# segasai/rvspecfit

Hardware: AMD Instinct MI355X
Metric: spectra/sec (CCF+chi2 grid) DESI 3-arm (higher is better)
Workload: dtype f64

## Files before the change

### include/rvsgpu.h

```cpp
#ifndef RVSGPU_H
#define RVSGPU_H
#include <stdint.h>

#ifdef __cplusplus
extern "C" {
#endif

#define RVS_E_ARG (-1)
#define RVS_E_LAUNCH (-2)

#define RVS_ST_SPLINE_RANGE 0x1
#define RVS_ST_SPLINE_GRID 0x2
#define RVS_ST_NONFINITE 0x4
#define RVS_ST_CHOL_FALLBACK 0x8
#define RVS_ST_OUTSIDE_NAN 0x10
#define RVS_ST_CCF_FAILED 0x20
#define RVS_ST_ALLMASKED 0x40
#define RVS_ST_QUAD_ASSERT 0x80
#define RVS_ST_ILLCOND 0x100
#define RVS_ST_NONPOS_MEDIAN 0x200
#define RVS_ST_RBF_NOTPD 0x400

#define RVS_ABI_VERSION 18
int rvs_abi_version(void);
// ... 80 lines not shown
int rvs_chisq_grid(const double *lam, const double *polysT, const double *work,
                   int npix, int npoly, int S, const double *knots,
                   const double *coef, int ntp, int Tn, int log_step,
                   const int32_t *job_spec, const int32_t *job_templ, int J,
                   const double *vels, int64_t vel_stride, int Nv,
                   const double *penalty, double badchi, double beta,
                   int pack_min_jobs, double *out, int32_t *status,
                   void *stream);

int64_t rvs_chisq_work_size_g(int npix, int S, int G);
int rvs_chisq_prepare_g(const double *lam, const double *spec,
                        const double *espec, int npix, int S, int G,
                        const double *knots_host3, int log_step, double espec_sys,
                        double *work, void *stream);
int rvs_chisq_grid_g(const double *lam, const double *polysT, const double *work,
                     int npix, int npoly, int S, const int32_t *grid_id, int G,
                     int64_t polys_stride, const double *knots,
                     const double *coef, int ntp, int Tn, int log_step,
                     const int32_t *job_spec, const int32_t *job_templ, int J,
                     const double *vels, int64_t vel_stride, int Nv,
                     const double *penalty, double badchi, double beta,
                     int pack_min_jobs, const double *pen_scale, double *out,
                     int32_t *status, void *stream);

int rvs_chisq_grid_resol(const double *lam, const double *polysT,
                         const double *work, int npix, int npoly, int S,
                         const double *knots, const double *coef, int ntp,
                         int Tn, int log_step, const double *taps, int nd,
                         int64_t taps_stride, const int32_t *job_spec,
                         const int32_t *job_templ, int J, const double *vels,
                         int64_t vel_stride, int Nv, const double *penalty,
                         double badchi, double beta, double *out,
                         int32_t *status, void *stream);
int rvs_chisq_grid_resol_g(const double *lam, const double *polysT,
                           const double *work, int npix, int npoly, int S,
                           const int32_t *grid_id, int G, int64_t polys_stride,
                           const double *knots, const double *coef, int ntp,
                           int Tn, int log_step, const double *taps, int nd,
                           int64_t taps_stride, const int32_t *job_spec,
                           const int32_t *job_templ, int J, const double *vels,
                           int64_t vel_stride, int Nv, const double *penalty,
                           double badchi, double beta, const double *pen_scale,
                           double *out, int32_t *status, void *stream);

int rvs_chisq_full(const double *lam, const double *polysT, const double *spec,
                   const double *espec, const uint8_t *badmask, int npix,
// ... 521 lines not shown
```

### rvspecfit_amd/_lib.py

```python
import ctypes
import os

import torch

_HERE = os.path.dirname(os.path.abspath(__file__))
LIB_PATH = os.path.join(_HERE, 'librvsgpu.so')

P = ctypes.c_void_p
I = ctypes.c_int
L = ctypes.c_int64
D = ctypes.c_double
U = ctypes.c_uint32

SIGNATURES = {
    'rvs_abi_version': (I, []),
    'rvs_option_set': (I, [ctypes.c_char_p, I]),
    'rvs_option_get': (I, [ctypes.c_char_p, P]),
    'rvs_template_polylinear': (I, [P, L, I, P, P, P, I, P, P, U, I, P, I, P, P,
                                    P, P, P]),
    'rvs_template_polylinear_grad': (I, [P, L, I, P, P, P, I, P, P, U, I, P, I, P,
                                         P, P, P, P]),
    'rvs_template_tri': (I, [P, I, P, P, P, I, I, U, I, P, I, P, P, P, P, P]),
    'rvs_template_tri_buckets': (I, [P, I, P, P, P, I, I, U, I, P, P, I, P, P, P,
                                     P, P]),
    'rvs_template_tri_grad': (I, [P, I, P, P, P, I, I, U, I, P, I, P, P, P, P, P]),
    'rvs_template_tri_buckets_grad': (I, [P, I, P, P, P, I, I, U, I, P, P, I, P, P,
                                          P, P, P]),
    'rvs_vsini_convolve': (I, [P, P, P, D, D, I, I, P, P]),
    'rvs_vsini_convolve_grad': (I, [P, P, P, D, D, I, I, I, P, P]),
    'rvs_spline_factors': (I, [P, I, P, P]),
    'rvs_spline_factors_len': (ctypes.c_int64, [I]),
    'rvs_spline_construct': (I, [P, P, I, I, I, P, P, P]),
    'rvs_spline_eval': (I, [P, P, I, I, P, I, I, P, P, P, P]),
    'rvs_chisq_work_size': (L, [I, I]),
    'rvs_chisq_work_size_g': (L, [I, I, I]),
    'rvs_chisq_prepare_g': (I, [P, P, P, I, I, I, P, I, D, P, P]),
    'rvs_chisq_grid_g': (I, [P, P, P, I, I, I, P, I, L, P, P, I, I, I, P, P, I, P, L,
                             I, P, D, D, I, P, P, P, P]),
    'rvs_chisq_prepare': (I, [P, P, P, I, I, P, I, D, P, P]),
    'rvs_chisq_grid': (I, [P, P, P, I, I, I, P, P, I, I, I, P, P, I, P, L, I, P,
                           D, D, I, P, P, P]),
    'rvs_chisq_grid_resol': (I, [P, P, P, I, I, I, P, P, I, I, I, P, I, L, P, P,
                                 I, P, L, I, P, D, D, P, P, P]),
    'rvs_chisq_grid_resol_g': (I, [P, P, P, I, I, I, P, I, L, P, P, I, I, I, P, I, L,
                                   P, P, I, P, L, I, P, D, D, P, P, P, P]),
    'rvs_chisq_full': (I, [P, P, P, P, P, I, I, I, P, P, I, I, I, I, I, P, P, I,
                           P, D, I, P, I, L, P, P, P, P, P, P, P, P]),
    'rvs_chisq_full_g': (I, [P, P, P, P, P, I, I, I, P, P, I, I, I, I, I, P, P, I,
                             P, D, I, P, I, L, P, P, P, P, P, P, P, P, I, L, P]),
    'rvs_chisq_continuum_work_size': (L, [I, I]),
    'rvs_chisq_continuum_g': (I, [P, P, P, P, P, I, I, I, P, P, P, P, P, P, I, L,
                                  P]),
    'rvs_chisq_continuum': (I, [P, P, P, P, P, I, I, I, P, P, P, P, P, P]),
    'rvs_chisq_point_work_size': (L, [I, I]),
    'rvs_chisq_point': (I, [P, I, I, P, P, I, P, D, P, P, P, P]),
    'rvs_chisq_point_grad_work_size': (L, [I, I, I]),
    'rvs_chisq_point_grad': (I, [P, I, I, I, P, P, I, P, D, P, P, P, P, P, P]),
    'rvs_chisq_point_fisher_work_size': (L, [I, I, I]),
    'rvs_chisq_point_fisher': (I, [P, I, I, I, P, P, I, P, D, P, P, P, P, P, P, P]),
    'rvs_chisq_point_grad_resol_work_size': (L, [I, I, I]),
    'rvs_chisq_point_grad_resol': (I, [P, I, I, I, P, P, I, P, D, P, P, P, P, P, P]),
# ... 309 lines not shown
```

### rvspecfit_amd/csrc/chisq.hip

```cpp
#include "common.h"
#include <type_traits>

extern "C" int64_t rvs_chisq_work_size_g(int npix, int S, int G) {
  return (int64_t)G * npix + 4ll * S * npix + 2ll * S + 2ll * G * npix;
}
extern "C" int64_t rvs_chisq_work_size(int npix, int S) {
  return rvs_chisq_work_size_g(npix, S, 1);
}

__global__ void __launch_bounds__(256)
    chisq_prepare_kernel(const double *__restrict__ lam,
                         const double *__restrict__ spec,
                         const double *__restrict__ espec, int npix, int S, int G,
                         double x0, double inv_step, int log_step,
                         double espec_sys, double *__restrict__ work) {
  __shared__ double red[8];
  const int s = blockIdx.x;
  double2 *W = reinterpret_cast<double2 *>(work + (int64_t)G * npix);
  double *scal = work + (int64_t)G * npix + 2ll * S * npix;
  double2 *X = reinterpret_cast<double2 *>(scal + 2ll * S);
  if (s >= S) {
    const double lx0 = log(x0);
    const double *lg = lam + (int64_t)(s - S) * npix;
    double *pixa = work + (int64_t)(s - S) * npix;
// ... 71 lines not shown
    if constexpr ((R & 1) != 0) asm volatile("" : "+s"(d));
  }
  __device__ __forceinline__ double get(int i) const {
    if (N8 >= 1 && i < 8) return a0[i];
    if (N8 >= 2 && i < 16) return a1[i - 8];
    int j = i - 8 * N8;
    if ((R & 4) != 0) {
      if (j < 4) return b[j];
      j -= 4;
    }
    if ((R & 2) != 0) {
      if (j < 2) return c[j];
      j -= 2;
    }
    return d;
  }
};
typedef int cg_v4i __attribute__((ext_vector_type(4)));
typedef int cg_v2i __attribute__((ext_vector_type(2)));
__device__ cg_v4i cg_sbl128(cg_v4i rsrc, int vindex, int voffset, int soffset,
                            int aux) __asm("llvm.amdgcn.struct.buffer.load.v4i32");
__device__ cg_v2i cg_sbl64(cg_v4i rsrc, int vindex, int voffset, int soffset,
                           int aux) __asm("llvm.amdgcn.struct.buffer.load.v2i32");
__device__ __forceinline__ cg_v4i cg_rsrc(const void *p, unsigned stride,
                                          unsigned nrec) {
  const unsigned long long a = (unsigned long long)p;
  cg_v4i r;
  r.x = (int)(unsigned)a;
  r.y = (int)(((unsigned)(a >> 32) & 0xffffu) | (stride << 16));
  r.z = (int)nrec;
  r.w = 0x00020000;
  return r;
}
template <int I, int N, class F>
__device__ __forceinline__ void cg_static_for(F &&f) {
  if constexpr (I < N) {
    f(std::integral_constant<int, I>{});
    cg_static_for<I + 1, N>(f);
  }
}
__device__ __forceinline__ void cg_sload2(double &d, const double *p) { d = *p; }
__device__ __forceinline__ void cg_sload4(cg_d2 &d, const double2 *p) {
  typedef double d2u __attribute__((ext_vector_type(2), aligned(8)));
  d = *reinterpret_cast<const d2u *>(p);
}

#define CG_WAVES(P) ((P) <= 10 ? 3 : 2)
__host__ __device__ constexpr int cg_split(int P) {
  if (P <= 13) return P;
  int pa = 1;
  while (pa < P && pa * (pa + 3) < P * (P + 3) / 2) pa++;
  return pa;
}

template <int P, bool TAIL>
__device__ __forceinline__ void
    chisq_grid_body(const int bx, const int by, const double *__restrict__ lam,
                      const double *__restrict__ polysT,
                      const double *__restrict__ work, int npix, int S,
                      const double *__restrict__ knots,
                      const double4 *__restrict__ coef, int ntp, int log_step,
                      const int32_t *__restrict__ job_spec,
                      const int32_t *__restrict__ job_templ, int J,
                      const double *__restrict__ vels, int64_t vel_stride,
                      int Nv, int iv0, int lpj,
                      const double *__restrict__ penalty, double badchi,
                      double beta_out, double *__restrict__ out,
                      int32_t *__restrict__ status, const GridSet GS) {
  int j, iv;
  bool active;
  if (TAIL) {
    const int64_t g = (int64_t)bx * 64 + threadIdx.x;
    j = (int)(g / lpj);
    iv = iv0 + (int)(g - (int64_t)j * lpj);
    active = j < J;
    if (!active) {
      j = 0;
      iv = iv0;
    }
  } else {
    j = by;
    iv = bx * 64 + threadIdx.x;
    active = iv < iv0;
    if (!active) iv = bx * 64;
  }
  const int s = job_spec ? job_spec[j] : j;
  const int t = job_templ ? job_templ[j] : j;
  double *outp = out + (int64_t)j * Nv;

  const double pen = penalty ? penalty[j] : 0.0;
  const bool unusable = !(pen == pen) || isinf(pen);
  if (GS.pen_scale) badchi *= GS.pen_scale[s];
  if (!TAIL && unusable) {
    if (active) {
      const double base = (beta_out != 0.0) ? beta_out * outp[iv] : 0.0;
      outp[iv] = base + 1000.0 * badchi;
    }
    return;
  }

  int gsel = 0;
  if (!TAIL && GS.gid) gsel = GS.gid[__builtin_amdgcn_readfirstlane(s)];
  gsel = __builtin_amdgcn_readfirstlane(gsel);
  lam += (int64_t)gsel * npix;
  polysT += (int64_t)gsel * GS.polys_stride;
  const double *pixa = work + (int64_t)gsel * npix;
  const double2 *W0 =
      reinterpret_cast<const double2 *>(work + (int64_t)GS.G * npix);
  const uint32_t woff = TAIL ? (uint32_t)s * (uint32_t)npix * 16u : 0u;
  const double2 *W = W0 + (TAIL ? 0 : (int64_t)s * npix);
  const double *scal = work + (int64_t)GS.G * npix + 2ll * S * npix + 2 * s;
  const double4 *cf = coef + (int64_t)t * ntp;

  const double vel = vels[(int64_t)j * vel_stride + iv];
  const double bb = vel / RVS_C_KMS;
  const double f = sqrt((1.0 - bb) / (1.0 + bb));
  const double x0 = knots[0], xlast = knots[ntp - 1];
  double shift;
  if (log_step) {
    const double inv_step = 1.0 / log(knots[1] / x0);
    shift = log(f) * inv_step;
  } else {
    shift = 0;
  }
  const double lin_inv_step = log_step ? 0.0 : 1.0 / (knots[1] - x0);

  int32_t st = 0;
  {
    const double xa = lam[0] * f, xb = lam[npix - 1] * f;
    if (xa < x0 || xb < x0 || xa >= xlast || xb >= xlast)
      st |= RVS_ST_SPLINE_RANGE;
  }
  int npx = npix;
  if (!TAIL && GS.gid) {
    const double last = lam[npix - 1];
    int lo = 0, hi = npix - 1;
    while (lo < hi) {
      const int mid = (lo + hi) >> 1;
      if (lam[mid] < last)
        lo = mid + 1;
      else
        hi = mid;
    }
    npx = __builtin_amdgcn_readfirstlane(lo + 1);
  }

  double acc[P * (P + 1) / 2];
  double av[P];
#pragma unroll
  for (int i = 0; i < P * (P + 1) / 2; i++) acc[i] = 0;
#pragma unroll
  for (int i = 0; i < P; i++) av[i] = 0;

  auto weights = [&](int k) -> double2 {
    if (TAIL)
      return *reinterpret_cast<const double2 *>(
          reinterpret_cast<const char *>(W0 + k) + woff);
    return W[k];
  };
  auto trips = [&](auto log_c, auto i0_c, auto i1_c) {
    constexpr bool LOG = decltype(log_c)::value;
    constexpr int I0 = decltype(i0_c)::value, I1 = decltype(i1_c)::value;
    auto pos_of = [&](double lamk, double pixk, double &x) {
      {
#pragma clang fp contract(off)
        x = lamk * f;
      }
      int pos;
      if (LOG)
        pos = (int)(pixk + shift);
      else
        pos = (int)((x - x0) * lin_inv_step);
      int r;
      asm("v_med3_i32 %0, %1, 0, %2" : "=v"(r) : "v"(pos), "s"(ntp - 2));
      return r;
    };
    const cg_v4i rk = cg_rsrc(knots, 8, (unsigned)ntp);
    const cg_v4i rc = cg_rsrc(cf, 32, (unsigned)ntp);
    auto knot_at = [&](int p) -> double {
      if (!TAIL) {
        const cg_v2i v = cg_sbl64(rk, p, 0, 0, 0);
        return __hiloint2double(v.y, v.x);
      }
      return *reinterpret_cast<const double *>(
          reinterpret_cast<const char *>(knots) + ((uint32_t)p << 3));
    };
    auto rec_at = [&](int p) -> double4 {
      if (!TAIL) {
        const cg_v4i lo = cg_sbl128(rc, p, 0, 0, 0);
        const cg_v4i hi = cg_sbl128(rc, p, 16, 0, 0);
        return make_double4(__hiloint2double(lo.y, lo.x),
                            __hiloint2double(lo.w, lo.z),
                            __hiloint2double(hi.y, hi.x),
                            __hiloint2double(hi.w, hi.z));
      }
      return *reinterpret_cast<const double4 *>(
          reinterpret_cast<const char *>(cf) + ((uint32_t)p << 5));
    };
    double w, u;
    {
      double x;
      const int p0 = pos_of(lam[0], pixa[0], x);
      const double d0 = x - knot_at(p0);
      const double4 c0 = rec_at(p0);
      const double2 w0 = weights(0);
      const double t0 = fma(fma(fma(c0.w, d0, c0.z), d0, c0.y), d0, c0.x);
      w = t0 * t0 * w0.x;
      u = t0 * w0.y;
    }
    const int klast = npx - 1;
    CgRow<P> R0, R1;
    double la0, pa0, la1, pa1;
    R0.load(polysT);
    cg_sload2(la0, lam + min(1, klast));
    cg_sload2(pa0, pixa + min(1, klast));
    asm volatile("" : "+s"(la0), "+s"(pa0));
    R0.pin();
    auto trip = [&](int k, CgRow<P> &Rc, CgRow<P> &Rn, double lac, double pac,
                    double &lan, double &pan) {
      const int k1 = min(k + 1, klast), k2 = min(k + 2, klast);
      Rn.load(polysT + (int64_t)k1 * P);
      cg_d2 wn_s;
      if (!TAIL) cg_sload4(wn_s, W + k1);
      cg_sload2(lan, lam + k2);
      cg_sload2(pan, pixa + k2);
      double xn;
      const int pn = pos_of(lac, pac, xn);
      double kn = knot_at(pn);
      double4 cn = rec_at(pn);
      double2 wn_v;
      if (TAIL) wn_v = weights(k1);
      CG_FENCE();
#pragma unroll
      for (int jj = 0; jj < I1; jj++) {
        const double pj = Rc.get(jj);
        const double pwj = pj * w;
        if (jj >= I0) av[jj] = fma(pj, u, av[jj]);
#pragma unroll
        for (int i = (jj > I0 ? jj : I0); i < I1; i++)
          acc[TRI(i, jj)] = fma(Rc.get(i), pwj, acc[TRI(i, jj)]);
      }
      CG_FENCE();
      asm volatile(""
                   : "+v"(kn), "+v"(cn.x), "+v"(cn.y), "+v"(cn.z), "+v"(cn.w));
      const double dn = xn - kn;
      const double tn = fma(fma(fma(cn.w, dn, cn.z), dn, cn.y), dn, cn.x);
      if (TAIL) {
        asm volatile("" : "+s"(lan), "+s"(pan));
        w = tn * tn * wn_v.x;
        u = tn * wn_v.y;
      } else {
        asm volatile("" : "+s"(lan), "+s"(pan), "+s"(wn_s));
        w = tn * tn * wn_s[0];
        u = tn * wn_s[1];
      }
      Rn.pin();
    };
    int k = 0;
#pragma unroll 1
    for (; k + 1 < npx; k += 2) {
      trip(k, R0, R1, la0, pa0, la1, pa1);
      trip(k + 1, R1, R0, la1, pa1, la0, pa0);
    }
    if (k < npx) trip(k, R0, R1, la0, pa0, la1, pa1);
  };
  constexpr int PS = cg_split(P);
  using c0_t = std::integral_constant<int, 0>;
  using cs_t = std::integral_constant<int, PS>;
  using cp_t = std::integral_constant<int, P>;
  if (log_step) {
    trips(std::true_type{}, c0_t{}, cs_t{});
    if constexpr (PS < P) trips(std::true_type{}, cs_t{}, cp_t{});
  } else {
    trips(std::false_type{}, c0_t{}, cs_t{});
    if constexpr (PS < P) trips(std::false_type{}, cs_t{}, cp_t{});
  }

  bool ok = true;
  double ldet = 0;
  double pmin = 1.79e308, pmax = 0;
#pragma unroll
  for (int i = 0; i < P; i++) {
#pragma unroll
    for (int jj = 0; jj <= i; jj++) {
      double sum = acc[TRI(i, jj)];
#pragma unroll
      for (int k = 0; k < jj; k++) sum -= acc[TRI(i, k)] * acc[TRI(jj, k)];
      if (jj == i) {
        if (!(sum > 0)) ok = false;
        pmin = fmin(pmin, sum);
        pmax = fmax(pmax, sum);
        const double d = sqrt(sum);
        acc[TRI(i, i)] = d;
// ... 54 lines not shown
  unsigned long long c0 = 0, r0 = 0;
  if (blockIdx.x == 4096) {
    c0 = __builtin_readcyclecounter();
    r0 = wall_clock64();
  }
#endif
  if (!TAIL) {
    const int per = 8 * nfull;
    const int g = bx / per, r = bx - g * per;
    by = g * 8 + (r & 7);
    bx = r >> 3;
    if (by >= J) return;
  }
  chisq_grid_body<P, TAIL>(bx, by, lam, polysT, work, npix, S,
                           knots, coef, ntp, log_step, job_spec, job_templ, J,
                           vels, vel_stride, Nv, iv0, lpj, penalty, badchi,
                           beta_out, out, status, GS);
#ifdef CG_CLOCK
  if (blockIdx.x == 4096 && threadIdx.x == 0) {
    cg_clock_dbg[0] = __builtin_readcyclecounter() - c0;
    cg_clock_dbg[1] = wall_clock64() - r0;
  }
#endif
}

#define RES_MAXND 33

template <int P>
__global__ void __launch_bounds__(256, (P <= 10 ? 2 : 1))
    chisq_grid_resol_kernel(const double *__restrict__ lam,
                            const double *__restrict__ polysT,
                            const double *__restrict__ work, int npix, int S,
                            const double *__restrict__ knots,
                            const double4 *__restrict__ coef, int ntp,
                            int log_step, const double *__restrict__ taps,
                            int nd, int64_t taps_stride,
                            const int32_t *__restrict__ job_spec,
                            const int32_t *__restrict__ job_templ,
                            const double *__restrict__ vels, int64_t vel_stride,
                            int Nv, const double *__restrict__ penalty,
                            double badchi, double beta_out,
                            double *__restrict__ out,
                            int32_t *__restrict__ status, GridSet GS) {
  extern __shared__ double ring[];
  const int j = blockIdx.y;
  const int wave_v0 = blockIdx.x * 256 + (threadIdx.x & ~63);
// ... 407 lines not shown
    }
    hipLaunchKernelGGL((chisq_grid_kernel<P, true>),
                       dim3((unsigned)(((int64_t)J * r + 63) / 64)),
                       dim3(64), 0, ts, lam, polysT, work, npix, S, knots, cf,
                       ntp, log_step, job_spec, job_templ, J, vels, vel_stride,
                       Nv, iv0, r, 0, penalty, badchi, beta, out, status, GS);
    RVS_LAUNCH_CHECK();
    if (fk && hipEventRecord(fk->join, fk->side) != hipSuccess)
      return RVS_E_LAUNCH;
  }
  if (nfull > 0) {
    const int64_t nb = (int64_t)((J + 7) / 8) * 8 * nfull;
    if (nb > 0x7fffffffll) return RVS_E_ARG;
    hipLaunchKernelGGL((chisq_grid_kernel<P, false>), dim3((unsigned)nb),
                       dim3(64), 0, st, lam, polysT, work, npix, S, knots, cf,
                       ntp, log_step, job_spec, job_templ, J, vels, vel_stride,
                       Nv, iv0, 64, nfull, penalty, badchi, beta, out, status,
                       GS);
    RVS_LAUNCH_CHECK();
  }
  if (fk && hipStreamWaitEvent(st, fk->join, 0) != hipSuccess)
    return RVS_E_LAUNCH;
  return 0;
}

extern "C" int rvs_chisq_prepare_g(const double *lam, const double *spec,
                                   const double *espec, int npix, int S, int G,
                                   const double *knots_host3, int log_step,
                                   double espec_sys, double *work, void *stream) {
  if (npix < 1 || S < 1 || G < 1 || !work) return RVS_E_ARG;
  const double x0 = knots_host3[0], x1 = knots_host3[1], x2 = knots_host3[2];
  double step, step2;
  if (log_step) {
    step = log(x1 / x0);
    step2 = log(x2 / x1);
  } else {
    step = x1 - x0;
    step2 = x2 - x1;
  }
  if (fabs(step - step2) > 1e-10) return -3;
  hipLaunchKernelGGL(chisq_prepare_kernel, dim3(S + G), dim3(256), 0,
                     rvs_stream(stream), lam, spec, espec, npix, S, G, x0,
                     1.0 / step, log_step, espec_sys, work);
  RVS_LAUNCH_CHECK();
  return 0;
}
// ... 1969 lines not shown
```

### rvspecfit_amd/csrc/options.cpp

```cpp
#include <atomic>
#include <cstdlib>
#include <cstring>
#include <mutex>

#include "options.h"

namespace {
struct OptDef {
  const char *name;
  const char *env;
  int dflt;
};
const OptDef kDefs[RVS_OPT_COUNT] = {
    {"xc_ws", "RVS_XC_WS", 1},
    {"obj_inblk_max", "RVS_OBJ_INBLK_MAX", 768},
    {"obj_sort", "RVS_OBJ_SORT", 1},
    {"nn_pipe", "RVS_NN_PIPE", 1},
    {"nm_split_min", "RVS_NM_SPLIT_MIN", 1024},
    {"nm_spec_max", "RVS_NM_SPEC_MAX", 21},
    {"nm_tail_window", "RVS_NM_TAIL_WINDOW", 16},
};
std::atomic<int> g_val[RVS_OPT_COUNT];
std::once_flag g_once;

void init_table() {
  for (int i = 0; i < RVS_OPT_COUNT; i++) {
    int v = kDefs[i].dflt;
    if (const char *ev = std::getenv(kDefs[i].env))
      v = std::atoi(ev);
    g_val[i].store(v, std::memory_order_relaxed);
  }
}
int find(const char *name) {
  if (!name) return -1;
  for (int i = 0; i < RVS_OPT_COUNT; i++)
    if (!std::strcmp(name, kDefs[i].name)) return i;
  return -1;
}
}

int rvs_opt(int id) {
  std::call_once(g_once, init_table);
  return g_val[id].load(std::memory_order_relaxed);
// ... 17 lines not shown
```

### rvspecfit_amd/csrc/options.h

```cpp
#pragma once
#include "../../include/rvsgpu.h"

enum {
  RVS_OPT_XC_WS,
  RVS_OPT_OBJ_INBLK_MAX,
  RVS_OPT_OBJ_SORT,
  RVS_OPT_NN_PIPE,
  RVS_OPT_NM_SPLIT_MIN,
  RVS_OPT_NM_SPEC_MAX,
  RVS_OPT_NM_TAIL_WINDOW,
  RVS_OPT_COUNT
};
int rvs_opt(int id);
```

### rvspecfit_amd/engine.py

```python
import numpy as np
import torch

from . import _lib
from . import ccf_tables

SPEED_OF_LIGHT = 299792.458

KTIMERS = None


class _ktime:

    def __init__(self, name, units=1):
        self.name, self.units = name, units

    def __enter__(self):
        if KTIMERS is not None:
            self.e0 = torch.cuda.Event(enable_timing=True)
            self.e0.record()

    def __exit__(self, *a):
        if KTIMERS is not None:
            e1 = torch.cuda.Event(enable_timing=True)
            e1.record()
# ... 535 lines not shown
    _lib.check(rc, 'rvs_spline_construct')
    if return_templ:
        return coef, outside, templ
    return coef, outside


def convolve_vsini(lib_or_lam, templ, vsini, eps=0.6):
    L = _lib.lib()
    lam = lib_or_lam.lam if hasattr(lib_or_lam, 'lam') else lib_or_lam
    ratios = lam[1:] / lam[:-1]
    assert np.allclose(ratios, ratios[0]), "Wavelength grid must be logarithmic."
    lnstep = float(np.log(ratios[0]))
    out = torch.empty_like(templ)
    rc = L.rvs_vsini_convolve(_lib.ptr(templ.contiguous()), _lib.ptr(vsini),
                              None, lnstep, float(eps), templ.shape[1],
                              templ.shape[0], _lib.ptr(out), _lib.stream())
    _lib.check(rc, 'rvs_vsini_convolve')
    return out


XCORR_PRUNE = True
import os as _os
CG_PACK_MIN_JOBS = 0


def _arm_resol(arm, ia, resols):
    if resols is not None and resols[ia] is not None:
        if arm.resol is not None:
            raise ValueError('You are not allowed to set resol_param together '
                             'with the resolution of each SpecData')
        return resols[ia]
    return arm.resol


def chisq_grid(batch, libs, coefs, outsides, vels, npoly=5, rbf=True,
               job_spec=None, job_templ=None, espec_sys=0.0,
               outside_penalty=True, out=None, vel_bounds=None, resols=None,
               defer_redo=False):
    L = _lib.lib()
    dev = batch.device
    if job_spec is not None:
        J = job_spec.shape[0]
    elif job_templ is not None:
        J = job_templ.shape[0]
    else:
        J = batch.S
    vels = vels.to(device=dev, dtype=torch.float64).contiguous()
    shared = vels.dim() == 1
    Nv = vels.shape[-1]
    vstride = 0 if shared else Nv
    def by_point_kernel(rows):
        js = job_spec if job_spec is not None else _arange32(0, J, dev)
        jt = job_templ if job_templ is not None else _arange32(0, J, dev)
        vv = vels[None, :].expand(J, Nv) if shared else vels
        if rows is not None:
            js, jt, vv = js[rows], jt[rows], vv[rows]
        n = js.shape[0]
        vv = vv.reshape(-1)
        res = torch.empty(n * Nv, dtype=torch.float64, device=dev)
        st = torch.zeros(n * Nv, dtype=torch.int32, device=dev)
        js2 = js.repeat_interleave(Nv).contiguous()
        jt2 = jt.repeat_interleave(Nv).contiguous()
# ... 25 lines not shown
            res[bad] = tot
            stb = torch.where(torch.isfinite(tot), stb,
                              stb | _lib.ST_NONFINITE)
            st[bad] = stb | _lib.ST_CHOL_FALLBACK
        stj = torch.zeros(n, dtype=torch.int32, device=dev)
        st = st.reshape(n, Nv)
        for bit in range(12):
            stj |= ((st >> bit) & 1).amax(dim=1).to(torch.int32) << bit
        return res.reshape(n, Nv), stj

    wide = [_arm_resol(arm, ia, resols) for ia, arm in enumerate(batch.arms)]
    if npoly > POINT_MAXP or \
            any(r is not None and r['nd'] > RES_MAXND for r in wide):
        res, stj = by_point_kernel(None)
        if out is not None:
            out.copy_(res)
            res = out
        return res, stj
    if out is None:
        out = torch.empty((J, Nv), dtype=torch.float64, device=dev)
    status = torch.zeros(J, dtype=torch.int32, device=dev)
    if vel_bounds is None:
        vel_bounds = (float(vels.min().item()), float(vels.max().item()))
    for ia, arm in enumerate(batch.arms):
        lib = libs[arm.name]
        work = arm.work(lib, espec_sys)
        polysT, logdet_off = arm.basis_ortho(npoly, rbf)
        o = outsides[ia]
        if job_templ is not None:
            o = o[job_templ.long()]
        pen = o * batch.badchi_jobs(job_spec) if outside_penalty else torch.where(
            torch.isfinite(o), torch.zeros_like(o), o)
        if torch.is_tensor(logdet_off):
            logdet_off = logdet_off if job_spec is None else \
                logdet_off[job_spec.long()]
        pen = (pen + logdet_off).contiguous()
        coef = coefs[ia]
        rs = _arm_resol(arm, ia, resols)
        for a, b in _chunks(J, 65535):
          with _ktime('chisq_grid', (b - a) * Nv):
            js = _lib.ptr(job_spec[a:b]) if job_spec is not None else \
                (_lib.ptr(_arange32(a, b, dev)) if a > 0 else None)
            jt = _lib.ptr(job_templ[a:b]) if job_templ is not None else \
                (_lib.ptr(_arange32(a, b, dev)) if a > 0 else None)
            if rs is not None:
                gid, G = arm.grid_args()
                rc = L.rvs_chisq_grid_resol_g(
                    _lib.ptr(arm.lam), _lib.ptr(polysT), _lib.ptr(work),
                    arm.npix, npoly, arm.S, gid, G, arm.basis_stride(npoly),
                    _lib.ptr(lib.knots), _lib.ptr(coef),
                    lib.ntp, coef.shape[0], int(lib.log_step),
                    _lib.ptr(rs['taps']), rs['nd'], rs['stride'], js, jt, b - a,
                    _lib.ptr(vels if shared else vels[a:b]), vstride, Nv,
                    _lib.ptr(pen[a:b]), float(batch.badchi),
                    0.0 if ia == 0 else 1.0, _lib.ptr(batch.pen_scale),
                    _lib.ptr(out[a:b]), _lib.ptr(status[a:b]), _lib.stream())
                _lib.check(rc, 'rvs_chisq_grid_resol')
                continue
            gid, G = arm.grid_args()
            rc = L.rvs_chisq_grid_g(
                _lib.ptr(arm.lam), _lib.ptr(polysT), _lib.ptr(work), arm.npix,
                npoly, arm.S, gid, G, arm.basis_stride(npoly),
                _lib.ptr(lib.knots), _lib.ptr(coef), lib.ntp,
                coef.shape[0], int(lib.log_step), js, jt, b - a,
                _lib.ptr(vels if shared else vels[a:b]), vstride, Nv,
                _lib.ptr(pen[a:b]), float(batch.badchi),
                0.0 if ia == 0 else 1.0, CG_PACK_MIN_JOBS,
                _lib.ptr(batch.pen_scale), _lib.ptr(out[a:b]),
                _lib.ptr(status[a:b]), _lib.stream())
            _lib.check(rc, 'rvs_chisq_grid')
    def finish():
        redo = torch.nonzero(status & (_lib.ST_ILLCOND | _lib.ST_CHOL_FALLBACK)
                             ).reshape(-1)
        if redo.numel():
            res, stj = by_point_kernel(redo)
            out[redo] = res
            status[redo] = (status[redo] & ~(_lib.ST_NONFINITE |
                                             _lib.ST_CHOL_FALLBACK)) | stj | \
                _lib.ST_ILLCOND
        return int(redo.numel())
    if defer_redo:
        return out, status, finish
    finish()
    return out, status


POINT_MAXP = 16
GRAD_MAXTAN = 6
GRAD_RESOL_LDS_MAX = 56 * 1024


def _per_arm(v, n):
    if isinstance(v, (list, tuple)):
# ... 548 lines not shown
```

Measured before the change: 78330.

## Precompute resampled template table per node and velocity for chi2 grid

```diff
diff --git a/include/rvsgpu.h b/include/rvsgpu.h
--- a/include/rvsgpu.h
+++ b/include/rvsgpu.h
@@ -126,6 +126,22 @@
                      const double *penalty, double badchi, double beta,
                      int pack_min_jobs, const double *pen_scale, double *out,
                      int32_t *status, void *stream);
+
+int64_t rvs_chisq_grid_tab_work_size(int npix, int Tn, int Nv, int64_t J_call,
+                                     int min_jobs_per_node, int pack_min_jobs);
+int rvs_chisq_grid_tab(const double *lam, const double *polysT, const double *work,
+                       int npix, int npoly, int S, const int32_t *grid_id, int G,
+                       int64_t polys_stride, const double *knots,
+                       const double *coef, int ntp, int Tn, int log_step,
+                       const int32_t *job_spec, const int32_t *job_templ, int J,
+                       const double *vels, int64_t vel_stride, int Nv,
+                       const double *penalty, double badchi, double beta,
+                       int pack_min_jobs, const double *pen_scale, double *out,
+                       int32_t *status, const int32_t *order,
+                       const int32_t *node_start, const int32_t *call_start,
+                       int64_t J_call, int min_jobs_per_node, double *tab,
+                       int64_t tab_size, int tab_state, int32_t *took,
+                       void *stream);
 
 int rvs_chisq_grid_resol(const double *lam, const double *polysT,
                          const double *work, int npix, int npoly, int S,
diff --git a/rvspecfit_amd/_lib.py b/rvspecfit_amd/_lib.py
--- a/rvspecfit_amd/_lib.py
+++ b/rvspecfit_amd/_lib.py
@@ -37,6 +37,9 @@
     'rvs_chisq_prepare_g': (I, [P, P, P, I, I, I, P, I, D, P, P]),
     'rvs_chisq_grid_g': (I, [P, P, P, I, I, I, P, I, L, P, P, I, I, I, P, P, I, P, L,
                              I, P, D, D, I, P, P, P, P]),
+    'rvs_chisq_grid_tab_work_size': (L, [I, I, I, L, I, I]),
+    'rvs_chisq_grid_tab': (I, [P, P, P, I, I, I, P, I, L, P, P, I, I, I, P, P, I, P, L,
+                               I, P, D, D, I, P, P, P, P, P, P, L, I, P, L, I, P, P]),
     'rvs_chisq_prepare': (I, [P, P, P, I, I, P, I, D, P, P]),
     'rvs_chisq_grid': (I, [P, P, P, I, I, I, P, P, I, I, I, P, P, I, P, L, I, P,
                            D, D, I, P, P, P]),
diff --git a/rvspecfit_amd/csrc/chisq.hip b/rvspecfit_amd/csrc/chisq.hip
--- a/rvspecfit_amd/csrc/chisq.hip
+++ b/rvspecfit_amd/csrc/chisq.hip
@@ -117,6 +117,8 @@
                             int aux) __asm("llvm.amdgcn.struct.buffer.load.v4i32");
 __device__ cg_v2i cg_sbl64(cg_v4i rsrc, int vindex, int voffset, int soffset,
                            int aux) __asm("llvm.amdgcn.struct.buffer.load.v2i32");
+__device__ cg_v2i cg_rbl64(cg_v4i rsrc, int voffset, int soffset,
+                           int aux) __asm("llvm.amdgcn.raw.buffer.load.v2i32");
 __device__ __forceinline__ cg_v4i cg_rsrc(const void *p, unsigned stride,
                                           unsigned nrec) {
   const unsigned long long a = (unsigned long long)p;
@@ -140,6 +142,74 @@
   d = *reinterpret_cast<const d2u *>(p);
 }
 
+__device__ __forceinline__ void cg_velocity(double vel,
+                                            const double *__restrict__ knots,
+                                            int log_step, double &f, double &shift,
+                                            double &lin_inv_step) {
+  const double bb = vel / RVS_C_KMS;
+  f = sqrt((1.0 - bb) / (1.0 + bb));
+  const double x0 = knots[0];
+  if (log_step) {
+    const double inv_step = 1.0 / log(knots[1] / x0);
+    shift = log(f) * inv_step;
+  } else {
+    shift = 0;
+  }
+  lin_inv_step = log_step ? 0.0 : 1.0 / (knots[1] - x0);
+}
+template <bool TAIL>
+__device__ __forceinline__ double cg_knot_at(const cg_v4i rk,
+                                             const double *__restrict__ knots,
+                                             int p) {
+  if (!TAIL) {
+    const cg_v2i v = cg_sbl64(rk, p, 0, 0, 0);
+    return __hiloint2double(v.y, v.x);
+  }
+  return *reinterpret_cast<const double *>(
+      reinterpret_cast<const char *>(knots) + ((uint32_t)p << 3));
+}
+template <bool TAIL>
+__device__ __forceinline__ double4 cg_rec_at(const cg_v4i rc,
+                                             const double4 *__restrict__ cf,
+                                             int p) {
+  if (!TAIL) {
+    const cg_v4i lo = cg_sbl128(rc, p, 0, 0, 0);
+    const cg_v4i hi = cg_sbl128(rc, p, 16, 0, 0);
+    return make_double4(__hiloint2double(lo.y, lo.x),
+                        __hiloint2double(lo.w, lo.z),
+                        __hiloint2double(hi.y, hi.x),
+                        __hiloint2double(hi.w, hi.z));
+  }
+  return *reinterpret_cast<const double4 *>(
+      reinterpret_cast<const char *>(cf) + ((uint32_t)p << 5));
+}
+template <bool LOG, bool TAIL, bool PIN, class Between>
+__device__ __forceinline__ double
+    cg_resample(double lamk, double pixk, double f, double shift, double x0,
+                double lin_inv_step, int ntp2, const cg_v4i rk,
+                const double *__restrict__ knots, const cg_v4i rc,
+                const double4 *__restrict__ cf, Between &&between) {
+  double x;
+  {
+#pragma clang fp contract(off)
+    x = lamk * f;
+  }
+  int pos;
+  if (LOG)
+    pos = (int)(pixk + shift);
+  else
+    pos = (int)((x - x0) * lin_inv_step);
+  int r;
+  asm("v_med3_i32 %0, %1, 0, %2" : "=v"(r) : "v"(pos), "s"(ntp2));
+  double kn = cg_knot_at<TAIL>(rk, knots, r);
+  double4 cn = cg_rec_at<TAIL>(rc, cf, r);
+  between();
+  if (PIN)
+    asm volatile("" : "+v"(kn), "+v"(cn.x), "+v"(cn.y), "+v"(cn.z), "+v"(cn.w));
+  const double dn = x - kn;
+  return fma(fma(fma(cn.w, dn, cn.z), dn, cn.y), dn, cn.x);
+}
+
 #define CG_WAVES(P) ((P) <= 10 ? 3 : 2)
 __host__ __device__ constexpr int cg_split(int P) {
   if (P <= 13) return P;
@@ -148,7 +218,8 @@
   return pa;
 }
 
-template <int P, bool TAIL>
+#define CG_TAB_AHEAD 4
+template <int P, bool TAIL, bool TAB = false>
 __device__ __forceinline__ void
     chisq_grid_body(const int bx, const int by, const double *__restrict__ lam,
                       const double *__restrict__ polysT,
@@ -161,7 +232,9 @@
                       int Nv, int iv0, int lpj,
                       const double *__restrict__ penalty, double badchi,
                       double beta_out, double *__restrict__ out,
-                      int32_t *__restrict__ status, const GridSet GS) {
+                      int32_t *__restrict__ status, const GridSet GS,
+                      const double *__restrict__ tstream = nullptr) {
+  static_assert(!(TAB && TAIL), "the node table serves full waves only");
   int j, iv;
   bool active;
   if (TAIL) {
@@ -208,17 +281,9 @@
   const double4 *cf = coef + (int64_t)t * ntp;
 
   const double vel = vels[(int64_t)j * vel_stride + iv];
-  const double bb = vel / RVS_C_KMS;
-  const double f = sqrt((1.0 - bb) / (1.0 + bb));
   const double x0 = knots[0], xlast = knots[ntp - 1];
-  double shift;
-  if (log_step) {
-    const double inv_step = 1.0 / log(knots[1] / x0);
-    shift = log(f) * inv_step;
-  } else {
-    shift = 0;
-  }
-  const double lin_inv_step = log_step ? 0.0 : 1.0 / (knots[1] - x0);
+  double f, shift, lin_inv_step;
+  cg_velocity(vel, knots, log_step, f, shift, lin_inv_step);
 
   int32_t st = 0;
   {
@@ -256,50 +321,14 @@
   auto trips = [&](auto log_c, auto i0_c, auto i1_c) {
     constexpr bool LOG = decltype(log_c)::value;
     constexpr int I0 = decltype(i0_c)::value, I1 = decltype(i1_c)::value;
-    auto pos_of = [&](double lamk, double pixk, double &x) {
-      {
-#pragma clang fp contract(off)
-        x = lamk * f;
-      }
-      int pos;
-      if (LOG)
-        pos = (int)(pixk + shift);
-      else
-        pos = (int)((x - x0) * lin_inv_step);
-      int r;
-      asm("v_med3_i32 %0, %1, 0, %2" : "=v"(r) : "v"(pos), "s"(ntp - 2));
-      return r;
-    };
     const cg_v4i rk = cg_rsrc(knots, 8, (unsigned)ntp);
     const cg_v4i rc = cg_rsrc(cf, 32, (unsigned)ntp);
-    auto knot_at = [&](int p) -> double {
-      if (!TAIL) {
-        const cg_v2i v = cg_sbl64(rk, p, 0, 0, 0);
-        return __hiloint2double(v.y, v.x);
-      }
-      return *reinterpret_cast<const double *>(
-          reinterpret_cast<const char *>(knots) + ((uint32_t)p << 3));
-    };
-    auto rec_at = [&](int p) -> double4 {
-      if (!TAIL) {
-        const cg_v4i lo = cg_sbl128(rc, p, 0, 0, 0);
-        const cg_v4i hi = cg_sbl128(rc, p, 16, 0, 0);
-        return make_double4(__hiloint2double(lo.y, lo.x),
-                            __hiloint2double(lo.w, lo.z),
-                            __hiloint2double(hi.y, hi.x),
-                            __hiloint2double(hi.w, hi.z));
-      }
-      return *reinterpret_cast<const double4 *>(
-          reinterpret_cast<const char *>(cf) + ((uint32_t)p << 5));
-    };
     double w, u;
     {
-      double x;
-      const int p0 = pos_of(lam[0], pixa[0], x);
-      const double d0 = x - knot_at(p0);
-      const double4 c0 = rec_at(p0);
-      const double2 w0 = weights(0);
-      const double t0 = fma(fma(fma(c0.w, d0, c0.z), d0, c0.y), d0, c0.x);
+      double2 w0;
+      const double t0 = cg_resample<LOG, TAIL, false>(
+          lam[0], pixa[0], f, shift, x0, lin_inv_step, ntp - 2, rk, knots, rc,
+          cf, [&]() { w0 = weights(0); });
       w = t0 * t0 * w0.x;
       u = t0 * w0.y;
     }
@@ -319,27 +348,22 @@
       if (!TAIL) cg_sload4(wn_s, W + k1);
       cg_sload2(lan, lam + k2);
       cg_sload2(pan, pixa + k2);
-      double xn;
-      const int pn = pos_of(lac, pac, xn);
-      double kn = knot_at(pn);
-      double4 cn = rec_at(pn);
       double2 wn_v;
-      if (TAIL) wn_v = weights(k1);
-      CG_FENCE();
-#pragma unroll
-      for (int jj = 0; jj < I1; jj++) {
-        const double pj = Rc.get(jj);
-        const double pwj = pj * w;
-        if (jj >= I0) av[jj] = fma(pj, u, av[jj]);
-#pragma unroll
-        for (int i = (jj > I0 ? jj : I0); i < I1; i++)
-          acc[TRI(i, jj)] = fma(Rc.get(i), pwj, acc[TRI(i, jj)]);
-      }
-      CG_FENCE();
-      asm volatile(""
-                   : "+v"(kn), "+v"(cn.x), "+v"(cn.y), "+v"(cn.z), "+v"(cn.w));
-      const double dn = xn - kn;
-      const double tn = fma(fma(fma(cn.w, dn, cn.z), dn, cn.y), dn, cn.x);
+      const double tn = cg_resample<LOG, TAIL, true>(
+          lac, pac, f, shift, x0, lin_inv_step, ntp - 2, rk, knots, rc, cf, [&]() {
+            if (TAIL) wn_v = weights(k1);
+            CG_FENCE();
+#pragma unroll
+            for (int jj = 0; jj < I1; jj++) {
+              const double pj = Rc.get(jj);
+              const double pwj = pj * w;
+              if (jj >= I0) av[jj] = fma(pj, u, av[jj]);
+#pragma unroll
+              for (int i = (jj > I0 ? jj : I0); i < I1; i++)
+                acc[TRI(i, jj)] = fma(Rc.get(i), pwj, acc[TRI(i, jj)]);
+            }
+            CG_FENCE();
+          });
       if (TAIL) {
         asm volatile("" : "+s"(lan), "+s"(pan));
         w = tn * tn * wn_v.x;
@@ -359,11 +383,79 @@
     }
     if (k < npx) trip(k, R0, R1, la0, pa0, la1, pa1);
   };
+  auto trips_tab = [&](auto i0_c, auto i1_c) {
+    constexpr int I0 = decltype(i0_c)::value, I1 = decltype(i1_c)::value;
+    constexpr int D = CG_TAB_AHEAD;
+    static_assert(D == 4, "the unrolled trips below are written for 4 slots");
+    const int klast = npx - 1;
+    const cg_v4i rt = cg_rsrc(tstream, 0, (unsigned)npix * 512u);
+    const int lo8 = (int)threadIdx.x * 8;
+    auto t_at = [&](int k) -> double {
+      const cg_v2i v = cg_rbl64(rt, lo8, min(k, klast) * 512, 0);
+      return __hiloint2double(v.y, v.x);
+    };
+    double q[D];
+#pragma unroll
+    for (int d = 0; d < D; d++) q[d] = t_at(d);
+    double w, u;
+    {
+      const double2 w0 = W[0];
+      const double t0 = q[0];
+      w = t0 * t0 * w0.x;
+      u = t0 * w0.y;
+    }
+    CgRow<P> R0, R1;
+    R0.load(polysT);
+    R0.pin();
+    auto trip = [&](int k, auto slot_c, CgRow<P> &Rc, CgRow<P> &Rn) {
+      constexpr int SL = decltype(slot_c)::value;
+      const int k1 = min(k + 1, klast);
+      Rn.load(polysT + (int64_t)k1 * P);
+      cg_d2 wn_s;
+      cg_sload4(wn_s, W + k1);
+      q[SL] = t_at(k + D);
+      CG_FENCE();
+#pragma unroll
+      for (int jj = 0; jj < I1; jj++) {
+        const double pj = Rc.get(jj);
+        const double pwj = pj * w;
+        if (jj >= I0) av[jj] = fma(pj, u, av[jj]);
+#pragma unroll
+        for (int i = (jj > I0 ? jj : I0); i < I1; i++)
+          acc[TRI(i, jj)] = fma(Rc.get(i), pwj, acc[TRI(i, jj)]);
+      }
+      CG_FENCE();
+      double tn = q[(SL + 1) % D];
+      asm volatile("" : "+v"(tn));
+      asm volatile("" : "+s"(wn_s));
+      w = tn * tn * wn_s[0];
+      u = tn * wn_s[1];
+      Rn.pin();
+    };
+    using s0_t = std::integral_constant<int, 0>;
+    using s1_t = std::integral_constant<int, 1>;
+    using s2_t = std::integral_constant<int, 2>;
+    using s3_t = std::integral_constant<int, 3>;
+    int k = 0;
+#pragma unroll 1
+    for (; k + 3 < npx; k += 4) {
+      trip(k, s0_t{}, R0, R1);
+      trip(k + 1, s1_t{}, R1, R0);
+      trip(k + 2, s2_t{}, R0, R1);
+      trip(k + 3, s3_t{}, R1, R0);
+    }
+    if (k < npx) trip(k, s0_t{}, R0, R1);
+    if (k + 1 < npx) trip(k + 1, s1_t{}, R1, R0);
+    if (k + 2 < npx) trip(k + 2, s2_t{}, R0, R1);
+  };
   constexpr int PS = cg_split(P);
   using c0_t = std::integral_constant<int, 0>;
   using cs_t = std::integral_constant<int, PS>;
   using cp_t = std::integral_constant<int, P>;
-  if (log_step) {
+  if constexpr (TAB) {
+    trips_tab(c0_t{}, cs_t{});
+    if constexpr (PS < P) trips_tab(cs_t{}, cp_t{});
+  } else if (log_step) {
     trips(std::true_type{}, c0_t{}, cs_t{});
     if constexpr (PS < P) trips(std::true_type{}, cs_t{}, cp_t{});
   } else {
@@ -464,6 +556,82 @@
     cg_clock_dbg[1] = wall_clock64() - r0;
   }
 #endif
+}
+
+#define CG_TAB_CHUNK 32
+__global__ void __launch_bounds__(64)
+    chisq_resample_kernel(const double *__restrict__ lam,
+                          const double *__restrict__ work, int npix,
+                          const double *__restrict__ knots,
+                          const double4 *__restrict__ coef, int ntp, int log_step,
+                          const double *__restrict__ vels, int nfull,
+                          const int32_t *__restrict__ node_start,
+                          double *__restrict__ tab) {
+  const int n = blockIdx.z, vb = blockIdx.y;
+  if (node_start[n + 1] == node_start[n]) return;
+  const double *pixa = work;
+  const double4 *cf = coef + (int64_t)n * ntp;
+  const double x0 = knots[0];
+  double f, shift, lin_inv_step;
+  cg_velocity(vels[vb * 64 + (int)threadIdx.x], knots, log_step, f, shift,
+              lin_inv_step);
+  const cg_v4i rk = cg_rsrc(knots, 8, (unsigned)ntp);
+  const cg_v4i rc = cg_rsrc(cf, 32, (unsigned)ntp);
+  double *o = tab + ((int64_t)n * nfull + vb) * npix * 64 + threadIdx.x;
+  const int ka = blockIdx.x * CG_TAB_CHUNK, kb = min(ka + CG_TAB_CHUNK, npix);
+  auto fill = [&](auto log_c) {
+    constexpr bool LOG = decltype(log_c)::value;
+    for (int k = ka; k < kb; k++)
+      o[(int64_t)k * 64] = cg_resample<LOG, false, false>(
+          lam[k], pixa[k], f, shift, x0, lin_inv_step, ntp - 2, rk, knots, rc, cf,
+          []() {});
+  };
+  if (log_step)
+    fill(std::true_type{});
+  else
+    fill(std::false_type{});
+}
+
+template <int P>
+__global__ void __launch_bounds__(64) __attribute__((amdgpu_waves_per_eu(
+    CG_WAVES(P))))
+    chisq_grid_tab_kernel(const double *__restrict__ lam,
+                          const double *__restrict__ polysT,
+                          const double *__restrict__ work, int npix, int S,
+                          const double *__restrict__ knots,
+                          const double4 *__restrict__ coef, int ntp, int log_step,
+                          const int32_t *__restrict__ job_spec,
+                          const int32_t *__restrict__ job_templ, int J,
+                          const double *__restrict__ vels, int Nv, int iv0,
+                          int nfull, const double *__restrict__ penalty,
+                          double badchi, double beta_out,
+                          double *__restrict__ out, int32_t *__restrict__ status,
+                          const GridSet GS, const int32_t *__restrict__ order,
+                          const int32_t *__restrict__ node_start, int Tn,
+                          const double *__restrict__ tab) {
+  const int64_t Q = (int64_t)nfull * J, per = (Q + 7) / 8;
+  const int64_t slot = blockIdx.x >> 3;
+  const int64_t item = (int64_t)(blockIdx.x & 7) * per + slot;
+  if (slot >= per || item >= Q) return;
+  int lo = 0, hi = Tn;
+  while (hi - lo > 1) {
+    const int mid = (lo + hi) >> 1;
+    if ((int64_t)node_start[mid] * nfull <= item)
+      lo = mid;
+    else
+      hi = mid;
+  }
+  const int n = __builtin_amdgcn_readfirstlane(lo);
+  const int s0 = node_start[n], nj = node_start[n + 1] - s0;
+  const int r = (int)(item - (int64_t)s0 * nfull);
+  if (nj < 1 || r < 0 || s0 < 0 || s0 + nj > J) return;
+  const int vb = r / nj;
+  const int j = __builtin_amdgcn_readfirstlane(order[s0 + (r - vb * nj)]);
+  if (vb >= nfull || (unsigned)j >= (unsigned)J) return;
+  chisq_grid_body<P, false, true>(
+      vb, j, lam, polysT, work, npix, S, knots, coef, ntp, log_step, job_spec,
+      job_templ, J, vels, 0, Nv, iv0, 64, penalty, badchi, beta_out, out, status,
+      GS, tab + ((int64_t)n * nfull + vb) * npix * 64);
 }
 
 #define RES_MAXND 33
@@ -917,6 +1085,115 @@
   if (fk && hipStreamWaitEvent(st, fk->join, 0) != hipSuccess)
     return RVS_E_LAUNCH;
   return 0;
+}
+
+#define CG_TAB_MAX_BYTES (1ll << 30)
+#define CG_TAB_MIN_JOBS_PER_NODE 16
+extern "C" int64_t rvs_chisq_grid_tab_work_size(int npix, int Tn, int Nv,
+                                                int64_t J_call,
+                                                int min_jobs_per_node,
+                                                int pack_min_jobs) {
+  if (min_jobs_per_node == 0) min_jobs_per_node = CG_TAB_MIN_JOBS_PER_NODE;
+  if (npix < 1 || Tn < 1 || Nv < 64 || J_call < 1 || min_jobs_per_node < 0 ||
+      (min_jobs_per_node > 1 && J_call < (int64_t)min_jobs_per_node * Tn) ||
+      !rvs_opt(RVS_OPT_CG_TAB))
+    return 0;
+  if (Nv % 64 != 0 && (pack_min_jobs < 0 || Nv % 64 > CG_PACK_MAXR)) return 0;
+  const int64_t n = (int64_t)Tn * (Nv / 64) * npix * 64;
+  return n * 8 <= CG_TAB_MAX_BYTES ? n : 0;
+}
+
+template <int P>
+static int launch_grid_tab(const double *lam, const double *polysT,
+                           const double *work, int npix, int S,
+                           const double *knots, const double *coef, int ntp,
+                           int Tn, int log_step, const int32_t *job_spec,
+                           const int32_t *job_templ, int J, const double *vels,
+                           int Nv, const double *penalty, double badchi,
+                           double beta, double *out, int32_t *status,
+                           const GridSet GS, const int32_t *order,
+                           const int32_t *node_start, const int32_t *call_start,
+                           double *tab, int tab_state, hipStream_t st) {
+  const int r = Nv % 64, nfull = Nv / 64, iv0 = Nv - r;
+  const double4 *cf = reinterpret_cast<const double4 *>(coef);
+  GridFork *fk = r ? grid_fork() : nullptr;
+  if (r) {
+    hipStream_t ts = st;
+    if (fk) {
+      if (hipEventRecord(fk->fork, st) != hipSuccess ||
+          hipStreamWaitEvent(fk->side, fk->fork, 0) != hipSuccess)
+        return RVS_E_LAUNCH;
+      ts = fk->side;
+    }
+    hipLaunchKernelGGL((chisq_grid_kernel<P, true>),
+                       dim3((unsigned)(((int64_t)J * r + 63) / 64)),
+                       dim3(64), 0, ts, lam, polysT, work, npix, S, knots, cf,
+                       ntp, log_step, job_spec, job_templ, J, vels, 0, Nv, iv0, r,
+                       0, penalty, badchi, beta, out, status, GS);
+    RVS_LAUNCH_CHECK();
+    if (fk && hipEventRecord(fk->join, fk->side) != hipSuccess)
+      return RVS_E_LAUNCH;
+  }
+  if (!tab_state) {
+    hipLaunchKernelGGL(chisq_resample_kernel,
+                       dim3((unsigned)((npix + CG_TAB_CHUNK - 1) / CG_TAB_CHUNK),
+                            (unsigned)nfull, (unsigned)Tn),
+                       dim3(64), 0, st, lam, work, npix, knots, cf, ntp, log_step,
+                       vels, nfull, call_start, tab);
+    RVS_LAUNCH_CHECK();
+  }
+  const int64_t nb = (((int64_t)nfull * J + 7) / 8) * 8;
+  hipLaunchKernelGGL((chisq_grid_tab_kernel<P>), dim3((unsigned)nb), dim3(64), 0,
+                     st, lam, polysT, work, npix, S, knots, cf, ntp, log_step,
+                     job_spec, job_templ, J, vels, Nv, iv0, nfull, penalty, badchi,
+                     beta, out, status, GS, order, node_start, Tn, tab);
+  RVS_LAUNCH_CHECK();
+  if (fk && hipStreamWaitEvent(st, fk->join, 0) != hipSuccess)
+    return RVS_E_LAUNCH;
+  return 0;
+}
+
+extern "C" int rvs_chisq_grid_tab(
+    const double *lam, const double *polysT, const double *work, int npix,
+    int npoly, int S, const int32_t *grid_id, int G, int64_t polys_stride,
+    const double *knots, const double *coef, int ntp, int Tn, int log_step,
+    const int32_t *job_spec, const int32_t *job_templ, int J, const double *vels,
+    int64_t vel_stride, int Nv, const double *penalty, double badchi, double beta,
+    int pack_min_jobs, const double *pen_scale, double *out, int32_t *status,
+    const int32_t *order, const int32_t *node_start, const int32_t *call_start,
+    int64_t J_call, int min_jobs_per_node, double *tab, int64_t tab_size,
+    int tab_state, int32_t *took, void *stream) {
+  if (took) *took = 0;
+  const int64_t need = rvs_chisq_grid_tab_work_size(
+      npix, Tn, Nv, J_call, min_jobs_per_node, pack_min_jobs);
+  const bool take =
+      job_templ && order && node_start && call_start && tab && vel_stride == 0 &&
+      G == 1 && !grid_id && J >= 1 && ntp >= 3 && npoly >= 1 && npoly <= 16 &&
+      need > 0 && need <= tab_size && J_call >= J &&
+      (Nv % 64 == 0 || (int64_t)S * npix * 16 < (1ll << 32)) &&
+      (int64_t)(Nv / 64) * J + 7 <= 0x7fffffffll;
+  if (!take)
+    return rvs_chisq_grid_g(lam, polysT, work, npix, npoly, S, grid_id, G,
+                            polys_stride, knots, coef, ntp, Tn, log_step, job_spec,
+                            job_templ, J, vels, vel_stride, Nv, penalty, badchi,
+                            beta, pack_min_jobs, pen_scale, out, status, stream);
+  if (took) *took = 1;
+  hipStream_t st = rvs_stream(stream);
+  const GridSet GS = {nullptr, polys_stride, 1, pen_scale};
+#define RVS_CASE(PP)                                                           \
+  case PP:                                                                     \
+    return launch_grid_tab<PP>(lam, polysT, work, npix, S, knots, coef, ntp, Tn, \
+                               log_step, job_spec, job_templ, J, vels, Nv,     \
+                               penalty, badchi, beta, out, status, GS, order,  \
+                               node_start, call_start, tab, tab_state, st);
+  switch (npoly) {
+    RVS_CASE(1) RVS_CASE(2) RVS_CASE(3) RVS_CASE(4) RVS_CASE(5) RVS_CASE(6)
+    RVS_CASE(7) RVS_CASE(8) RVS_CASE(9) RVS_CASE(10) RVS_CASE(11) RVS_CASE(12)
+    RVS_CASE(13) RVS_CASE(14) RVS_CASE(15) RVS_CASE(16)
+    default:
+      return RVS_E_ARG;
+  }
+#undef RVS_CASE
 }
 
 extern "C" int rvs_chisq_prepare_g(const double *lam, const double *spec,
diff --git a/rvspecfit_amd/csrc/options.cpp b/rvspecfit_amd/csrc/options.cpp
--- a/rvspecfit_amd/csrc/options.cpp
+++ b/rvspecfit_amd/csrc/options.cpp
@@ -19,6 +19,7 @@
     {"nm_split_min", "RVS_NM_SPLIT_MIN", 1024},
     {"nm_spec_max", "RVS_NM_SPEC_MAX", 21},
     {"nm_tail_window", "RVS_NM_TAIL_WINDOW", 16},
+    {"cg_tab", "RVS_CG_TAB", 1},
 };
 std::atomic<int> g_val[RVS_OPT_COUNT];
 std::once_flag g_once;
diff --git a/rvspecfit_amd/csrc/options.h b/rvspecfit_amd/csrc/options.h
--- a/rvspecfit_amd/csrc/options.h
+++ b/rvspecfit_amd/csrc/options.h
@@ -9,6 +9,7 @@
   RVS_OPT_NM_SPLIT_MIN,
   RVS_OPT_NM_SPEC_MAX,
   RVS_OPT_NM_TAIL_WINDOW,
+  RVS_OPT_CG_TAB,
   RVS_OPT_COUNT
 };
 int rvs_opt(int id);
diff --git a/rvspecfit_amd/engine.py b/rvspecfit_amd/engine.py
--- a/rvspecfit_amd/engine.py
+++ b/rvspecfit_amd/engine.py
@@ -1,3 +1,6 @@
+import ctypes
+import threading
+
 import numpy as np
 import torch
 
@@ -581,6 +584,16 @@
 XCORR_PRUNE = True
 import os as _os
 CG_PACK_MIN_JOBS = 0
+CG_TAB_MIN_JOBS = 0
+_cg_tab_tls = threading.local()
+
+
+def cg_tab_took():
+    return getattr(_cg_tab_tls, 'took', 0)
+
+
+def _cg_tab_work(dev, n):
+    return torch.empty(n, dtype=torch.float64, device=dev)
 
 
 def _arm_resol(arm, ia, resols):
@@ -597,6 +610,7 @@
                outside_penalty=True, out=None, vel_bounds=None, resols=None,
                defer_redo=False):
     L = _lib.lib()
+    _cg_tab_tls.took = 0
     dev = batch.device
     if job_spec is not None:
         J = job_spec.shape[0]
@@ -668,6 +682,28 @@
     status = torch.zeros(J, dtype=torch.int32, device=dev)
     if vel_bounds is None:
         vel_bounds = (float(vels.min().item()), float(vels.max().item()))
+    tab = None
+    took = ctypes.c_int32(0)
+    ntook = 0
+    if job_templ is not None and shared and Nv >= 64 and CG_TAB_MIN_JOBS >= 0 \
+            and all(r is None for r in wide) \
+            and all(a.grid_args()[1] == 1 for a in batch.arms):
+        Tn = coefs[0].shape[0]
+        ntab = max(L.rvs_chisq_grid_tab_work_size(a.npix, c.shape[0], Nv, J,
+                                                  CG_TAB_MIN_JOBS,
+                                                  CG_PACK_MIN_JOBS)
+                   for a, c in zip(batch.arms, coefs))
+        if all(c.shape[0] == Tn for c in coefs) and ntab > 0:
+            nodes = torch.arange(Tn + 1, dtype=torch.int32, device=dev)
+
+            def by_node(jt):
+                srt, order = torch.sort(jt, stable=True)
+                start = torch.searchsorted(srt, nodes, out_int32=True)
+                return order.to(torch.int32).contiguous(), start.contiguous()
+            tab_chunks = [by_node(job_templ[a:b]) for a, b in _chunks(J, 65535)]
+            tab_call = tab_chunks[0][1] if len(tab_chunks) == 1 else \
+                by_node(job_templ)[1]
+            tab = _cg_tab_work(dev, ntab)
     for ia, arm in enumerate(batch.arms):
         lib = libs[arm.name]
         work = arm.work(lib, espec_sys)
@@ -683,7 +719,7 @@
         pen = (pen + logdet_off).contiguous()
         coef = coefs[ia]
         rs = _arm_resol(arm, ia, resols)
-        for a, b in _chunks(J, 65535):
+        for ic, (a, b) in enumerate(_chunks(J, 65535)):
           with _ktime('chisq_grid', (b - a) * Nv):
             js = _lib.ptr(job_spec[a:b]) if job_spec is not None else \
                 (_lib.ptr(_arange32(a, b, dev)) if a > 0 else None)
@@ -704,6 +740,24 @@
                 _lib.check(rc, 'rvs_chisq_grid_resol')
                 continue
             gid, G = arm.grid_args()
+            if tab is not None:
+                order, start = tab_chunks[ic]
+                rc = L.rvs_chisq_grid_tab(
+                    _lib.ptr(arm.lam), _lib.ptr(polysT), _lib.ptr(work), arm.npix,
+                    npoly, arm.S, gid, G, arm.basis_stride(npoly),
+                    _lib.ptr(lib.knots), _lib.ptr(coef), lib.ntp,
+                    coef.shape[0], int(lib.log_step), js, jt, b - a,
+                    _lib.ptr(vels), vstride, Nv,
+                    _lib.ptr(pen[a:b]), float(batch.badchi),
+                    0.0 if ia == 0 else 1.0, CG_PACK_MIN_JOBS,
+                    _lib.ptr(batch.pen_scale), _lib.ptr(out[a:b]),
+                    _lib.ptr(status[a:b]), _lib.ptr(order), _lib.ptr(start),
+                    _lib.ptr(tab_call), J, CG_TAB_MIN_JOBS, _lib.ptr(tab),
+                    tab.numel(), 1 if ic else 0, ctypes.byref(took),
+                    _lib.stream())
+                _lib.check(rc, 'rvs_chisq_grid_tab')
+                ntook += took.value
+                continue
             rc = L.rvs_chisq_grid_g(
                 _lib.ptr(arm.lam), _lib.ptr(polysT), _lib.ptr(work), arm.npix,
                 npoly, arm.S, gid, G, arm.basis_stride(npoly),
@@ -715,6 +769,7 @@
                 _lib.ptr(batch.pen_scale), _lib.ptr(out[a:b]),
                 _lib.ptr(status[a:b]), _lib.stream())
             _lib.check(rc, 'rvs_chisq_grid')
+    _cg_tab_tls.took = ntook
     def finish():
         redo = torch.nonzero(status & (_lib.ST_ILLCOND | _lib.ST_CHOL_FALLBACK)
                              ).reshape(-1)
```

Measured after the change: 84380, median of 6. +7.7%, better.
